# lgen-sudo/EgoM2P

Measured on AMD Instinct MI355X. Metric: multimodal tokens/sec (ego-b 400M, 10300-tok clips), training fwd+bwd+allreduce+AdamW, higher is better.
Workload: dtype bf16; 1 GPU; egom2p_base_12e_12d_swiglu_nobias mod4, synthetic 10300-position clips (1009+1009 rgb, 1009+1009 depth, 15+15 cam, 15+15 gaze kept -> N=M=2048), bf16 MFMA GEMM/attention, fp32 residual/LN/CE/AdamW; micro_batch=64, global_batch=256, parallelism=dp1

## Files before the change

egom2p_amd/csrc/gemm.hip:

```cpp
#include "common.h"
#include "egom2p_hip.h"

namespace {

constexpr int BM = 128, BN = 128, BK = 64;
constexpr int TILE_BYTES = BM * BK * 2;
constexpr int STAGE_BYTES = 2 * TILE_BYTES;
constexpr int GEMM_LDS = 2 * STAGE_BYTES;
constexpr int EPI_BYTES = 16 * 1024;
constexpr int NT_LDS = GEMM_LDS + EPI_BYTES;

struct NTArgs {
    const bf16_t* A; long lda;
    const bf16_t* B; long ldb;
    void* C; long ldc;
    const float* R; long ldr;
    const float* bias;
    const int* m_range;
    int M, N, K, epi;
    const bf16_t* X; long ldx;
    bf16_t* H; long ldh;
    const float* sa; const float* sb;
    int dephase;
};
// ... 124 lines not shown
                    for (int i = 0; i < 4; ++i) {
                        const int ml = i * 16 + (lane & 15);
#pragma unroll
                        for (int j = 0; j < 4; ++j) {
                            const int c = wn * 16 + j * 4 + (lane >> 4);
                            *(f32x4*)(ebuf + ml * 512 + ((c ^ (ml & 15)) << 4)) = acc[i][j];
                        }
                    }
                }
                lds_barrier();
#pragma unroll
                for (int ps = 0; ps < 8; ++ps) {
                    const int r = ps * 8 + (tid >> 5), c = tid & 31;
                    f32x4 v = *(const f32x4*)(ebuf + r * 512 + ((c ^ (r & 15)) << 4));
                    const int gm = row0 + half * 64 + r, gn = col0 + c * 4;
                    if (gm < M && gn < p.N) {
                        const long mrow = moff + gm;
                        if (p.epi == EGO_EPI_RESID) {
                            const f32x4 rr = *(const f32x4*)(p.R + mrow * p.ldr + gn);
                            v = f32x4{rr[0] + round_bf16(v[0]), rr[1] + round_bf16(v[1]), rr[2] + round_bf16(v[2]), rr[3] + round_bf16(v[3])};
                        } else if (p.epi == EGO_EPI_BIAS_RESID) {
                            const f32x4 rr = *(const f32x4*)(p.R + mrow * p.ldr + gn);
                            const f32x4 b = *(const f32x4*)(p.bias + gn);
                            v = f32x4{rr[0] + round_bf16(v[0] + round_bf16(b[0])), rr[1] + round_bf16(v[1] + round_bf16(b[1])),
                                      rr[2] + round_bf16(v[2] + round_bf16(b[2])), rr[3] + round_bf16(v[3] + round_bf16(b[3]))};
                        }
                        *(f32x4*)((float*)p.C + mrow * p.ldc + gn) = v;
                    }
                }
                lds_barrier();
            }
        }
        if (!more) break;
        tile = next_tile;
    }
}

template <int TM, int TN, int NS>
struct NTL {
    static constexpr int PA = TM / 32, PB = TN / 32;
    static constexpr int TA = TM * 128, TB = TN * 128;
    static constexpr int STAGE = TA + TB;
    static constexpr int LDS = NS * STAGE;
    static constexpr int PER = PA + PB;
};
constexpr int NT64_LDS = NTL<64, 64, 4>::LDS;
constexpr int NTL128x64_LDS = NTL<128, 64, 3>::LDS;
constexpr int NTL128x128_LDS = NTL<128, 128, 3>::LDS;

template <int N>
__device__ __forceinline__ void vm_wait() { asm volatile("s_waitcnt vmcnt(%0)" ::"n"(N) : "memory"); }

template <int TM, int TN, int NS>
__global__ __launch_bounds__(256, (NTL<TM, TN, NS>::LDS <= 80 * 1024 ? 2 : 1)) void gemm_ntl_kernel(NTArgs p) {
    using T = NTL<TM, TN, NS>;
    constexpr int MI = TM / 32, NI = TN / 32;
    extern __shared__ __attribute__((aligned(16))) char smem[];
    const int tid = threadIdx.x, lane = tid & 63;
    const int wave = __builtin_amdgcn_readfirstlane(tid >> 6);
    const int wm = wave >> 1, wn = wave & 1;
    int M = p.M;
    long moff = 0;
    if (p.m_range) { moff = p.m_range[0]; M = min(M, p.m_range[1]); }
    const int tiles_n = (p.N + TN - 1) / TN;
    const int tile = xcd_remap(blockIdx.x, gridDim.x);
    const int row0 = (tile / tiles_n) * TM, col0 = (tile % tiles_n) * TN;
    if (row0 >= M) return;
    const int nt = p.K / BK;

    const bf16_t* ga[T::PA];
    const bf16_t* gb[T::PB];
#pragma unroll
    for (int j = 0; j < T::PA; ++j) {
        const int r = 8 * (T::PA * wave + j) + (lane >> 3);
        ga[j] = p.A + (moff + min(row0 + r, M - 1)) * p.lda + ((lane & 7) ^ (r & 7)) * 8;
    }
#pragma unroll
    for (int j = 0; j < T::PB; ++j) {
        const int r = 8 * (T::PB * wave + j) + (lane >> 3);
        gb[j] = p.B + (long)min(col0 + r, p.N - 1) * p.ldb + ((lane & 7) ^ (r & 7)) * 8;
    }
    auto stage = [&](int s, int k0) {
        char* sa = smem + s * T::STAGE + wave * T::PA * 1024;
        char* sb = smem + s * T::STAGE + T::TA + wave * T::PB * 1024;
#pragma unroll
        for (int j = 0; j < T::PA; ++j) glds16(ga[j] + k0, sa + j * 1024);
#pragma unroll
        for (int j = 0; j < T::PB; ++j) glds16(gb[j] + k0, sb + j * 1024);
    };
#pragma unroll
    for (int s = 0; s < NS - 1; ++s)
        if (s < nt) stage(s, s * BK);

    f32x4 acc[MI][NI];
#pragma unroll
    for (int i = 0; i < MI; ++i)
#pragma unroll
        for (int j = 0; j < NI; ++j) acc[i][j] = f32x4{0.f, 0.f, 0.f, 0.f};
    int cur = 0;
    for (int kt = 0; kt < nt; ++kt) {
        const int younger = min(nt - 1 - kt, NS - 2);
        if (NS >= 4 && younger >= 2) vm_wait<2 * T::PER>();
        else if (younger >= 1) vm_wait<T::PER>();
        else vm_wait<0>();
        lds_barrier();
        if (kt + NS - 1 < nt) stage(cur == 0 ? NS - 1 : cur - 1, (kt + NS - 1) * BK);
        const char* sa = smem + cur * T::STAGE;
        const char* sb = sa + T::TA;
#pragma unroll
        for (int ks = 0; ks < 2; ++ks) {
            bf16x8 af[MI], bfr[NI];
            const int c = ks * 4 + (lane >> 4);
#pragma unroll
            for (int i = 0; i < MI; ++i) {
                const int ar = wm * (TM / 2) + i * 16 + (lane & 15);
                af[i] = *(const bf16x8*)(sa + ar * 128 + ((c ^ (ar & 7)) << 4));
            }
#pragma unroll
            for (int j = 0; j < NI; ++j) {
                const int br = wn * (TN / 2) + j * 16 + (lane & 15);
                bfr[j] = *(const bf16x8*)(sb + br * 128 + ((c ^ (br & 7)) << 4));
            }
#pragma unroll
            for (int i = 0; i < MI; ++i)
#pragma unroll
                for (int j = 0; j < NI; ++j)
                    acc[i][j] = __builtin_amdgcn_mfma_f32_16x16x32_bf16(bfr[j], af[i], acc[i][j], 0, 0, 0);
        }
        cur = (cur + 1 == NS) ? 0 : cur + 1;
    }

#pragma unroll
    for (int i = 0; i < MI; ++i) {
        const int gm = row0 + wm * (TM / 2) + i * 16 + (lane & 15);
#pragma unroll
        for (int j = 0; j < NI; ++j) {
            const int gn = col0 + wn * (TN / 2) + j * 16 + 4 * (lane >> 4);
            if (gm >= M || gn >= p.N) continue;
            const long mrow = moff + gm;
            f32x4 v = acc[i][j];
            if (p.epi == EGO_EPI_BF16) {
                *(u32x2*)((bf16_t*)p.C + mrow * p.ldc + gn) = u32x2{pack_bf16x2(v[0], v[1]), pack_bf16x2(v[2], v[3])};
                continue;
            }
            if (p.epi == EGO_EPI_RESID) {
                const f32x4 rr = *(const f32x4*)(p.R + mrow * p.ldr + gn);
                v = f32x4{rr[0] + round_bf16(v[0]), rr[1] + round_bf16(v[1]), rr[2] + round_bf16(v[2]), rr[3] + round_bf16(v[3])};
            } else if (p.epi == EGO_EPI_BIAS_RESID) {
                const f32x4 rr = *(const f32x4*)(p.R + mrow * p.ldr + gn);
                const f32x4 b = *(const f32x4*)(p.bias + gn);
                v = f32x4{rr[0] + round_bf16(v[0] + round_bf16(b[0])), rr[1] + round_bf16(v[1] + round_bf16(b[1])),
                          rr[2] + round_bf16(v[2] + round_bf16(b[2])), rr[3] + round_bf16(v[3] + round_bf16(b[3]))};
            }
            *(f32x4*)((float*)p.C + mrow * p.ldc + gn) = v;
        }
    }
}
#define gemm_nt64_kernel (gemm_ntl_kernel<64, 64, 4>)

constexpr int T2_BYTES = 256 * 128;
constexpr int S2_BYTES = 2 * T2_BYTES;
constexpr int NT2_LDS = 2 * S2_BYTES;

__device__ __forceinline__ void bar_pinned() {
    __builtin_amdgcn_sched_barrier(0);
    __builtin_amdgcn_s_barrier();
    __builtin_amdgcn_sched_barrier(0);
}

#ifndef NT256_STRIPS
#define NT256_STRIPS 1
#endif
#ifndef NT256_A_AUX
#define NT256_A_AUX 0
#endif
#ifndef NT256_B_AUX
#define NT256_B_AUX 0
#endif
constexpr int RA_BYTES = 256 * 128;
constexpr int NT3_LDS = 5 * RA_BYTES;

typedef int i32x8 __attribute__((ext_vector_type(8)));
__device__ __forceinline__ i32x8 cat_frag(bf16x8 lo, bf16x8 hi) {
    typedef int i32x4 __attribute__((ext_vector_type(4)));
    const i32x4 a = __builtin_bit_cast(i32x4, lo), b = __builtin_bit_cast(i32x4, hi);
    return __builtin_shufflevector(a, b, 0, 1, 2, 3, 4, 5, 6, 7);
}

template <int EK, bool FP8 = false, bool STRIPS = false>
__global__ __launch_bounds__(512, 2) void gemm_nt256_kernel(NTArgs p) {
    constexpr int ESZ = FP8 ? 1 : 2;
    extern __shared__ __attribute__((aligned(16))) char smem[];
    const int tid = threadIdx.x, lane = tid & 63;
    const int wave = __builtin_amdgcn_readfirstlane(tid >> 6);
    const int grp = wave >> 2, wc = wave & 3;

    int M = p.M;
    long moff = 0;
    if (p.m_range) { moff = p.m_range[0]; M = min(M, p.m_range[1]); }
    if (M <= 0) return;
    const int tiles_n = EK == 3 ? p.N / 128 : (p.N + 255) / 256;
    const int tile_w = EK == 3 ? 128 : 256;
    const int ntiles = ((M + 255) / 256) * tiles_n;
    if ((int)blockIdx.x >= ntiles) return;
    const int nt = p.K * ESZ / 128;
    const int G = gridDim.x;
    if (p.dephase > 0 && ((blockIdx.x >> 3) & 1))
        for (int i = 0; i < p.dephase; ++i) __builtin_amdgcn_s_sleep(16);

    auto a_rsrc = [&](int row0) {
        return __builtin_amdgcn_make_buffer_rsrc((void*)((const char*)p.A + (moff + row0) * p.lda * ESZ), 0,
                                                 (int)(unsigned)((long)(min(256, M - row0) - 1) * p.lda * ESZ + (long)p.K * ESZ), 0x00020000);
    };
    const __amdgpu_buffer_rsrc_t brs = __builtin_amdgcn_make_buffer_rsrc(
        (void*)p.B, 0, (int)(unsigned)((long)((EK == 3 ? 2 * p.N : p.N) - 1) * p.ldb * ESZ + (long)p.K * ESZ), 0x00020000);
    unsigned a_off0, b_off0;
    {
        const int r = 8 * (wave * 4) + (lane >> 3), c = ((lane & 7) ^ (r & 7)) * 16;
        a_off0 = (unsigned)(r * (int)p.lda * ESZ + c);
        b_off0 = (unsigned)((EK == 3 && r >= 128 ? p.N - 128 + r : r) * (int)p.ldb * ESZ + c);
    }
    const unsigned a_step = (unsigned)(8 * (int)p.lda * ESZ), b_step = (unsigned)(8 * (int)p.ldb * ESZ);
    const int rows_t = (M + 255) / 256;
    const int nstrips = STRIPS ? (tiles_n + 7) / 8 : 1;
    const int w0 = tiles_n / nstrips, wide = tiles_n % nstrips;
    const int big = wide * (w0 + 1) * rows_t;
    auto tile_origin = [&](int id, int& row0, int& col0) {
        const int t = xcd_remap(id, ntiles);
        int tr, tc;
        if constexpr (STRIPS) {
            int rem, w, c0;
            if (t < big) { const int per = (w0 + 1) * rows_t, sidx = t / per; rem = t - sidx * per; w = w0 + 1; c0 = sidx * (w0 + 1); }
            else { const int per = w0 * rows_t, u = t - big, sidx = u / per; rem = u - sidx * per; w = w0; c0 = wide * (w0 + 1) + sidx * w0; }
            tr = rem / w; tc = c0 + rem % w;
        } else {
            tr = t / tiles_n; tc = t % tiles_n;
        }
        row0 = tr * 256; col0 = tc * tile_w;
    };
    int idA = blockIdx.x, ktA = 0, rA, cA_unused, slotA = 0; bool moreA = true;
    int idB = blockIdx.x, ktB = 0, rB_unused, cB, slotB = 0; bool moreB = true;
    tile_origin(idA, rA, cA_unused);
    tile_origin(idB, rB_unused, cB);
    unsigned a_so = 0, b_so = 0;
    __amdgpu_buffer_rsrc_t ars = a_rsrc(rA);
    auto cursorA = [&]() { a_so = (unsigned)(ktA * BK * 2); };
    auto advanceA = [&]() {
        slotA = slotA == 2 ? 0 : slotA + 1;
        if (++ktA == nt) {
            ktA = 0; idA += G;
            if (idA < ntiles) { tile_origin(idA, rA, cA_unused); ars = a_rsrc(rA); } else moreA = false;
        }
    };
    auto cursorB = [&]() { b_so = (unsigned)cB * (unsigned)(p.ldb * ESZ) + (unsigned)(ktB * BK * 2); };
    auto advanceB = [&]() {
        slotB ^= 1;
        if (++ktB == nt) { ktB = 0; idB += G; if (idB < ntiles) tile_origin(idB, rB_unused, cB); else moreB = false; }
    };
    auto dmaA = [&](int slot, int j) {
        __builtin_amdgcn_raw_ptr_buffer_load_lds(ars, (__attribute__((address_space(3))) void*)(smem + slot * RA_BYTES + (wave * 4 + j) * 1024),
                                                 16, a_off0, (int)(a_so + j * a_step), 0, NT256_A_AUX);
    };
    auto dmaB = [&](int slot, int j) {
        __builtin_amdgcn_raw_ptr_buffer_load_lds(brs, (__attribute__((address_space(3))) void*)(smem + (3 + slot) * RA_BYTES + (wave * 4 + j) * 1024),
                                                 16, b_off0, (int)(b_so + j * b_step), 0, NT256_B_AUX);
    };
#ifndef FP8_FRAG_OLD
#define FP8_FRAG_OLD 0
#endif
    int foff[2];
#pragma unroll
    for (int ks = 0; ks < 2; ++ks)
        foff[ks] = (lane & 15) * 128 + ((((FP8 && FP8_FRAG_OLD) ? 2 * (lane >> 4) + ks : ks * 4 + (lane >> 4)) ^ (lane & 7)) << 4);
    const int a_base = grp * 128 * 128, b_base = wc * 64 * 128;

    int id = blockIdx.x, row0, col0;
    tile_origin(id, row0, col0);
    cursorA();
#pragma unroll
    for (int j = 0; j < 4; ++j) dmaA(slotA, j);
    advanceA();
    cursorB();
#pragma unroll
    for (int j = 0; j < 4; ++j) dmaB(slotB, j);
    advanceB();
    if (moreA) {
        cursorA();
#pragma unroll
        for (int j = 0; j < 4; ++j) dmaA(slotA, j);
        advanceA();
        asm volatile("s_waitcnt vmcnt(4)" ::: "memory");
    } else {
        asm volatile("s_waitcnt vmcnt(0)" ::: "memory");
    }
    bar_pinned();
    int curA = 0, curB = 0;

#define LOAD_A(QM)                                                                                         \
    _Pragma("unroll") for (int mi = 0; mi < 4; ++mi) _Pragma("unroll") for (int ks = 0; ks < 2; ++ks)      \
        af[mi][ks] = *(const bf16x8*)(sa + a_base + ((QM) * 4 + mi) * 2048 + foff[ks]);
#define LOAD_B(QN)                                                                                         \
    _Pragma("unroll") for (int ni = 0; ni < 2; ++ni) _Pragma("unroll") for (int ks = 0; ks < 2; ++ks)      \
        bq[ni][ks] = *(const bf16x8*)(sb + b_base + ((QN) * 2 + ni) * 2048 + foff[ks]);
#define COMPUTE(QM, QN)                                                                                    \
    __builtin_amdgcn_s_setprio(1);                                                                         \
    if constexpr (FP8) {                                                                                   \
        _Pragma("unroll") for (int mi = 0; mi < 4; ++mi) _Pragma("unroll") for (int ni = 0; ni < 2; ++ni)  \
            acc[(QM) * 4 + mi][(QN) * 2 + ni] = __builtin_amdgcn_mfma_scale_f32_16x16x128_f8f6f4(          \
                cat_frag(bq[ni][0], bq[ni][1]), cat_frag(af[mi][0], af[mi][1]),                            \
                acc[(QM) * 4 + mi][(QN) * 2 + ni], 0, 0, 0, 127, 0, 127);                                  \
    } else {                                                                                               \
        _Pragma("unroll") for (int ks = 0; ks < 2; ++ks) _Pragma("unroll") for (int mi = 0; mi < 4; ++mi)  \
            _Pragma("unroll") for (int ni = 0; ni < 2; ++ni)                                               \
                acc[(QM) * 4 + mi][(QN) * 2 + ni] = __builtin_amdgcn_mfma_f32_16x16x32_bf16(               \
                    bq[ni][ks], af[mi][ks], acc[(QM) * 4 + mi][(QN) * 2 + ni], 0, 0, 0);                   \
    }                                                                                                      \
    __builtin_amdgcn_s_setprio(0);

    while (true) {
        f32x4 acc[8][4];
#pragma unroll
        for (int i = 0; i < 8; ++i)
#pragma unroll
            for (int j = 0; j < 4; ++j) acc[i][j] = f32x4{0.f, 0.f, 0.f, 0.f};
        bf16x8 af[4][2], bq[2][2];

        if (grp == 1) bar_pinned();
        for (int kt = 0; kt < nt; ++kt) {
            const char* sa = smem + curA * RA_BYTES;
            const char* sb = smem + (3 + curB) * RA_BYTES;
            const bool fa = moreA, fb = moreB;
            const int sA = slotA, sB = slotB;
            if (fa) cursorA();
            if (fb) cursorB();
            LOAD_A(0) LOAD_B(0)
            if (grp == 1) { if (fb) { dmaB(sB, 0); dmaB(sB, 1); } } else if (fa) { dmaA(sA, 0); dmaA(sA, 1); }
            bar_pinned();
            COMPUTE(0, 0)
            bar_pinned();
            LOAD_B(1)
            if (fb) { if (grp == 1) { dmaB(sB, 2); dmaB(sB, 3); } else { dmaB(sB, 0); dmaB(sB, 1); } }
            bar_pinned();
            COMPUTE(0, 1)
            bar_pinned();
            LOAD_A(1)
            if (grp == 1) { if (fa) { dmaA(sA, 0); dmaA(sA, 1); } } else if (fb) { dmaB(sB, 2); dmaB(sB, 3); }
            bar_pinned();
            COMPUTE(1, 1)
            bar_pinned();
            LOAD_B(0)
            if (fa) { dmaA(sA, 2); dmaA(sA, 3); }
            if (grp == 1) { if (fa) asm volatile("s_waitcnt vmcnt(4)" ::: "memory"); else asm volatile("s_waitcnt vmcnt(0)" ::: "memory"); }
            bar_pinned();
            COMPUTE(1, 0)
            if (grp == 0) { if (fa) asm volatile("s_waitcnt vmcnt(2)" ::: "memory"); else asm volatile("s_waitcnt vmcnt(0)" ::: "memory"); }
            bar_pinned();
            if (fa) advanceA();
            if (fb) advanceB();
            curA = curA == 2 ? 0 : curA + 1;
            curB ^= 1;
        }
        if (grp == 0) bar_pinned();
        asm volatile("s_waitcnt lgkmcnt(0)" ::: "memory");

        char* ea = smem + (curA == 0 ? 2 : curA - 1) * RA_BYTES;
        char* ebb = smem + (3 + (curB ^ 1)) * RA_BYTES;
        if constexpr (FP8) {
            float ra[8];
            f32x4 cb[4];
#pragma unroll
            for (int i = 0; i < 8; ++i) ra[i] = p.sa[moff + min(row0 + grp * 128 + i * 16 + (lane & 15), M - 1)];
#pragma unroll
            for (int j = 0; j < 4; ++j) {
                const int tc = wc * 64 + j * 16 + (lane >> 4) * 4;
                const int bn = EK == 3 ? (tc < 128 ? col0 + tc : p.N + col0 + tc - 128) : min(col0 + tc, p.N - 4);
                cb[j] = *(const f32x4*)(p.sb + bn);
            }
#pragma unroll
            for (int j = 0; j < 4; ++j)
#pragma unroll
                for (int i = 0; i < 8; ++i) acc[i][j] = acc[i][j] * (cb[j] * ra[i]);
        }
        if constexpr (EK == 0) {
#pragma unroll
            for (int half = 0; half < 2; ++half) {
                if (grp == half) {
    #pragma unroll
                    for (int i = 0; i < 8; ++i) {
                        const int ml = i * 16 + (lane & 15);
                        char* eb = (i < 4 ? ea : ebb) + (ml & 63) * 512;
    #pragma unroll
                        for (int j = 0; j < 4; ++j) {
                            const int slot = wc * 16 + j * 4 + (lane >> 4);
                            const f32x4 v = acc[i][j];
                            u32x2 o = {pack_bf16x2(v[0], v[1]), pack_bf16x2(v[2], v[3])};
                            *(u32x2*)(eb + (((slot >> 1) ^ (ml & 15)) << 4) + (slot & 1) * 8) = o;
                        }
                    }
                }
                lds_barrier();
    #pragma unroll
                for (int ps = 0; ps < 8; ++ps) {
                    const int r = ps * 16 + (tid >> 5), c = tid & 31;
                    const u32x4 v = *(const u32x4*)((ps < 4 ? ea : ebb) + (r & 63) * 512 + ((c ^ (r & 15)) << 4));
                    const int gm = row0 + half * 128 + r, gn = col0 + c * 8;
                    if (gm < M && gn < p.N) __builtin_nontemporal_store(v, (u32x4*)((bf16_t*)p.C + (moff + gm) * p.ldc + gn));
                }
                lds_barrier();
            }
        } else if constexpr (EK == 3) {
            bf16_t* Cb = (bf16_t*)p.C + moff * p.ldc;
            bf16_t* Hb = p.H + moff * p.ldh;
#pragma unroll
            for (int half = 0; half < 2; ++half) {
                if (grp == half) {
#pragma unroll
                    for (int i = 0; i < 8; ++i) {
                        const int ml = i * 16 + (lane & 15);
                        char* eb = (i < 4 ? ea : ebb) + (ml & 63) * 512;
#pragma unroll
                        for (int j = 0; j < 4; ++j) {
                            const int slot = wc * 16 + j * 4 + (lane >> 4);
                            const f32x4 v = acc[i][j];
                            u32x2 o = {pack_bf16x2(v[0], v[1]), pack_bf16x2(v[2], v[3])};
                            *(u32x2*)(eb + (((slot >> 1) ^ (ml & 15)) << 4) + (slot & 1) * 8) = o;
                        }
                    }
                }
                lds_barrier();
#pragma unroll
                for (int ps = 0; ps < 4; ++ps) {
                    const int r = ps * 32 + (tid >> 4), c = tid & 15;
                    const char* rowp = (ps < 2 ? ea : ebb) + (r & 63) * 512;
                    const u32x4 av = *(const u32x4*)(rowp + ((c ^ (r & 15)) << 4));
                    const u32x4 bv = *(const u32x4*)(rowp + (((c + 16) ^ (r & 15)) << 4));
                    u32x4 hv;
#pragma unroll
                    for (int e = 0; e < 4; ++e) {
                        const float a0 = bf16_to_f32(av[e] & 0xffff), a1 = bf16_to_f32(av[e] >> 16);
                        const float b0 = bf16_to_f32(bv[e] & 0xffff), b1 = bf16_to_f32(bv[e] >> 16);
                        hv[e] = pack_bf16x2(round_bf16(a0 * sigmoidf_(a0)) * b0, round_bf16(a1 * sigmoidf_(a1)) * b1);
                    }
                    const int gm = row0 + half * 128 + r, gn = col0 + c * 8;
                    if (gm < M) {
                        __builtin_nontemporal_store(av, (u32x4*)(Cb + (long)gm * p.ldc + gn));
                        __builtin_nontemporal_store(bv, (u32x4*)(Cb + (long)gm * p.ldc + p.N + gn));
                        __builtin_nontemporal_store(hv, (u32x4*)(Hb + (long)gm * p.ldh + gn));
                    }
                }
                lds_barrier();
            }
        } else if constexpr (EK == 2) {
            const bf16_t* Xb = p.X + moff * p.ldx;
            bf16_t* Yb = (bf16_t*)p.C + moff * p.ldc;
            auto load_ab = [&](int g, u32x4 (&av)[2], u32x4 (&bv)[2]) {
#pragma unroll
                for (int k = 0; k < 2; ++k) {
                    const int gm = row0 + (g >> 2) * 128 + ((g & 3) * 2 + k) * 16 + (tid >> 5), gn = col0 + (tid & 31) * 8;
                    const u32x4 z = {0u, 0u, 0u, 0u};
                    const bool ok = g < 8 && gm < M;
                    av[k] = ok ? __builtin_nontemporal_load((const u32x4*)(Xb + (long)gm * p.ldx + gn)) : z;
                    bv[k] = ok ? __builtin_nontemporal_load((const u32x4*)(Xb + (long)gm * p.ldx + p.N + gn)) : z;
                }
            };
            auto process = [&](int g, const u32x4 (&av)[2], const u32x4 (&bv)[2]) {
#pragma unroll
                for (int k = 0; k < 2; ++k) {
                    const int ps = (g & 3) * 2 + k;
                    const int r = ps * 16 + (tid >> 5), c = tid & 31;
                    const u32x4 gq = *(const u32x4*)((ps < 4 ? ea : ebb) + (r & 63) * 512 + ((c ^ (r & 15)) << 4));
                    const int gm = row0 + (g >> 2) * 128 + r, gn = col0 + c * 8;
                    u32x4 oa, ob;
#pragma unroll
                    for (int e = 0; e < 4; ++e) {
                        const float a2[2] = {bf16_to_f32(av[k][e] & 0xffff), bf16_to_f32(av[k][e] >> 16)};
                        const float b2[2] = {bf16_to_f32(bv[k][e] & 0xffff), bf16_to_f32(bv[k][e] >> 16)};
                        const float g2[2] = {bf16_to_f32(gq[e] & 0xffff), bf16_to_f32(gq[e] >> 16)};
                        float da[2], db[2];
#pragma unroll
                        for (int t = 0; t < 2; ++t) {
                            const float sg = sigmoidf_(a2[t]);
                            da[t] = g2[t] * b2[t] * sg * (1.f + a2[t] * (1.f - sg));
                            db[t] = g2[t] * a2[t] * sg;
                        }
                        oa[e] = pack_bf16x2(da[0], da[1]);
                        ob[e] = pack_bf16x2(db[0], db[1]);
                    }
                    if (gm < M) {
                        __builtin_nontemporal_store(oa, (u32x4*)(Yb + (long)gm * p.ldc + gn));
                        __builtin_nontemporal_store(ob, (u32x4*)(Yb + (long)gm * p.ldc + p.N + gn));
                    }
                }
            };
            u32x2 pk[8][4];
#pragma unroll
            for (int i = 0; i < 8; ++i)
#pragma unroll
                for (int j = 0; j < 4; ++j) {
                    const f32x4 v = acc[i][j];
                    pk[i][j] = u32x2{pack_bf16x2(v[0], v[1]), pack_bf16x2(v[2], v[3])};
                }
            u32x4 av[4][2], bv[4][2];
#pragma unroll
            for (int g = 0; g < 4; ++g) load_ab(g, av[g], bv[g]);
#pragma unroll
            for (int half = 0; half < 2; ++half) {
                if (grp == half) {
#pragma unroll
                    for (int i = 0; i < 8; ++i) {
                        const int ml = i * 16 + (lane & 15);
                        char* eb = (i < 4 ? ea : ebb) + (ml & 63) * 512;
#pragma unroll
                        for (int j = 0; j < 4; ++j) {
                            const int slot = wc * 16 + j * 4 + (lane >> 4);
                            *(u32x2*)(eb + (((slot >> 1) ^ (ml & 15)) << 4) + (slot & 1) * 8) = pk[i][j];
                        }
                    }
                }
                lds_barrier();
#pragma unroll
                for (int gg = 0; gg < 4; ++gg) {
                    const int g = half * 4 + gg;
                    process(g, av[gg], bv[gg]);
                    if (half == 0) load_ab(g + 4, av[gg], bv[gg]);
                }
                lds_barrier();
            }
        } else {
            const bool has_r = (p.epi == EGO_EPI_RESID || p.epi == EGO_EPI_BIAS_RESID);
            f32x4 bb = {0.f, 0.f, 0.f, 0.f};
            if (p.epi == EGO_EPI_BIAS_RESID) {
                const int gn = col0 + (tid & 63) * 4;
                if (gn < p.N) { const f32x4 b = *(const f32x4*)(p.bias + gn); bb = f32x4{round_bf16(b[0]), round_bf16(b[1]), round_bf16(b[2]), round_bf16(b[3])}; }
            }
            auto load_r = [&](int q, int hb, f32x4 (&rr)[4]) {
#pragma unroll
                for (int k = 0; k < 4; ++k) {
                    const int gm = row0 + q * 64 + (hb * 4 + k) * 8 + (tid >> 6), gn = col0 + (tid & 63) * 4;
                    rr[k] = (has_r && q < 4 && gm < M && gn < p.N) ? __builtin_nontemporal_load((const f32x4*)(p.R + (moff + gm) * p.ldr + gn))
                                                                    : f32x4{0.f, 0.f, 0.f, 0.f};
                }
            };
            f32x4 rlo[4], rhi[4];
            load_r(0, 0, rlo);
            load_r(0, 1, rhi);
#pragma unroll
            for (int q = 0; q < 4; ++q) {
                if (grp == (q >> 1)) {
#pragma unroll
                    for (int ii = 0; ii < 4; ++ii) {
                        const int i = (q & 1) * 4 + ii;
                        const int ml = ii * 16 + (lane & 15);
                        char* eb = (ii < 2 ? ea : ebb) + (ml & 31) * 1024;
#pragma unroll
                        for (int j = 0; j < 4; ++j) {
                            const int c = wc * 16 + j * 4 + (lane >> 4);
                            *(f32x4*)(eb + ((c ^ (ml & 15)) << 4)) = acc[i][j];
                        }
                    }
                }
                lds_barrier();
#pragma unroll
                for (int hb = 0; hb < 2; ++hb) {
                    f32x4 (&rr)[4] = hb == 0 ? rlo : rhi;
#pragma unroll
                    for (int k = 0; k < 4; ++k) {
                        const int r = (hb * 4 + k) * 8 + (tid >> 6), c = tid & 63;
                        f32x4 v = *(const f32x4*)((hb == 0 ? ea : ebb) + (r & 31) * 1024 + ((c ^ (r & 15)) << 4));
                        const int gm = row0 + q * 64 + r, gn = col0 + c * 4;
                        if (gm < M && gn < p.N) {
                            if (has_r) {
                                const f32x4 x = rr[k];
                                v = f32x4{x[0] + round_bf16(v[0] + bb[0]), x[1] + round_bf16(v[1] + bb[1]),
                                          x[2] + round_bf16(v[2] + bb[2]), x[3] + round_bf16(v[3] + bb[3])};
                            }
                            *(f32x4*)((float*)p.C + (moff + gm) * p.ldc + gn) = v;
                        }
                    }
                    if (q < 3) load_r(q + 1, hb, rr);
                }
                lds_barrier();
            }
        }
        id += G;
        if (id >= ntiles) break;
        tile_origin(id, row0, col0);
    }
#undef LOAD_A
#undef LOAD_B
#undef COMPUTE
}

struct TNArgs {
    const bf16_t* P; long ldp;
    const bf16_t* Q; long ldq;
    float* C0; float* C1; long ldc;
    float* slab;
    const int* m_range;
    int split_row, rows0, rows1;
    int Ni, Nj, M, splits;
};

__device__ __forceinline__ int tn_f(int r) { return (r & 3) | (((r >> 3) & 1) << 2); }


template <int S>
__device__ __forceinline__ void tn_compute(const unsigned (&pb)[4], const unsigned (&qb)[4], f32x4 (&acc)[4][4]) {
    constexpr int O = S * STAGE_BYTES;
    s16x4 p0[4][2], q0[4][2], p1[4][2], q1[4][2];
#pragma unroll
    for (int i = 0; i < 4; ++i) {
        p0[i][0] = tr_read<O>(pb[i]);              p0[i][1] = tr_read<O + 1024>(pb[i]);
        q0[i][0] = tr_read<O + TILE_BYTES>(qb[i]); q0[i][1] = tr_read<O + TILE_BYTES + 1024>(qb[i]);
    }
    asm volatile("s_waitcnt lgkmcnt(0)" ::: "memory");
    __builtin_amdgcn_sched_barrier(0);
#pragma unroll
    for (int i = 0; i < 4; ++i) {
        p1[i][0] = tr_read<O + 8192>(pb[i]);              p1[i][1] = tr_read<O + 8192 + 1024>(pb[i]);
        q1[i][0] = tr_read<O + TILE_BYTES + 8192>(qb[i]); q1[i][1] = tr_read<O + TILE_BYTES + 8192 + 1024>(qb[i]);
    }
    __builtin_amdgcn_sched_barrier(0);
#pragma unroll
    for (int i = 0; i < 4; ++i)
#pragma unroll
        for (int j = 0; j < 4; ++j)
            acc[i][j] = __builtin_amdgcn_mfma_f32_16x16x32_bf16(join8(q0[j][0], q0[j][1]), join8(p0[i][0], p0[i][1]), acc[i][j], 0, 0, 0);
    __builtin_amdgcn_sched_barrier(0);
    asm volatile("s_waitcnt lgkmcnt(0)" ::: "memory");
    __builtin_amdgcn_sched_barrier(0);
#pragma unroll
    for (int i = 0; i < 4; ++i)
#pragma unroll
        for (int j = 0; j < 4; ++j)
            acc[i][j] = __builtin_amdgcn_mfma_f32_16x16x32_bf16(join8(q1[j][0], q1[j][1]), join8(p1[i][0], p1[i][1]), acc[i][j], 0, 0, 0);
}

__global__ __launch_bounds__(256, 2) void gemm_tn_kernel(TNArgs p) {
    extern __shared__ __attribute__((aligned(16))) char smem[];
    const int tid = threadIdx.x, lane = tid & 63;
    const int wave = __builtin_amdgcn_readfirstlane(tid >> 6);
    const int wi = wave >> 1, wj = wave & 1;

    int M = p.M;
    long moff = 0;
    if (p.m_range) { moff = p.m_range[0]; M = min(M, p.m_range[1]); }
    const int tiles_j = p.Nj / BN, tiles_i = p.Ni / BM;
    const int ntile = tiles_i * tiles_j;
    const int bid = blockIdx.x;
    const int split = bid / ntile;
    const int t = xcd_remap(bid % ntile, ntile);
    const int i0 = (t / tiles_j) * BM, j0 = (t % tiles_j) * BN;

    const int nsteps = (M + BK - 1) / BK;
    const int per = (nsteps + p.splits - 1) / p.splits;
    const int st0 = split * per, st1 = min(nsteps, st0 + per);

    const bf16_t* P = p.P + moff * p.ldp + i0;
    const bf16_t* Q = p.Q + moff * p.ldq + j0;

    long p_off[4], q_off[4];
#pragma unroll
    for (int j = 0; j < 4; ++j) {
        const int r = 4 * (wave * 4 + j) + (lane >> 4), s16 = lane & 15;
        const int c = (((s16 >> 1) ^ tn_f(r)) << 1) | (s16 & 1);
// ... 488 lines not shown
```

Measured before the change: 1.964 million clip-positions/s.

## Interleave LDS reads and DMA issues between individual MFMAs in bf16 GEMM mainloop

For the bf16 path, the GEMM mainloop is rewritten as a hand-scheduled sequence. Each MFMA is followed by one LDS fragment read or global-to-LDS DMA issue, with sched_barrier pins between them. The next tile's first fragments are prefetched during the last quarter, and there are fewer workgroup barriers per k-step. The aim is to hide LDS latency and barrier stalls behind matrix math. This risks correctness hazards from the changed wait counts and barrier placement, plus extra register pressure. The FP8 path keeps the old loop.

```diff
diff --git a/egom2p_amd/csrc/gemm.hip b/egom2p_amd/csrc/gemm.hip
--- a/egom2p_amd/csrc/gemm.hip
+++ b/egom2p_amd/csrc/gemm.hip
@@ -450,20 +450,23 @@
 #define LOAD_B(QN)                                                                                         \
     _Pragma("unroll") for (int ni = 0; ni < 2; ++ni) _Pragma("unroll") for (int ks = 0; ks < 2; ++ks)      \
         bq[ni][ks] = *(const bf16x8*)(sb + b_base + ((QN) * 2 + ni) * 2048 + foff[ks]);
-#define COMPUTE(QM, QN)                                                                                    \
+#define COMPUTE(QM, QN)                          \
     __builtin_amdgcn_s_setprio(1);                                                                         \
-    if constexpr (FP8) {                                                                                   \
-        _Pragma("unroll") for (int mi = 0; mi < 4; ++mi) _Pragma("unroll") for (int ni = 0; ni < 2; ++ni)  \
-            acc[(QM) * 4 + mi][(QN) * 2 + ni] = __builtin_amdgcn_mfma_scale_f32_16x16x128_f8f6f4(          \
-                cat_frag(bq[ni][0], bq[ni][1]), cat_frag(af[mi][0], af[mi][1]),                            \
-                acc[(QM) * 4 + mi][(QN) * 2 + ni], 0, 0, 0, 127, 0, 127);                                  \
-    } else {                                                                                               \
-        _Pragma("unroll") for (int ks = 0; ks < 2; ++ks) _Pragma("unroll") for (int mi = 0; mi < 4; ++mi)  \
-            _Pragma("unroll") for (int ni = 0; ni < 2; ++ni)                                               \
-                acc[(QM) * 4 + mi][(QN) * 2 + ni] = __builtin_amdgcn_mfma_f32_16x16x32_bf16(               \
-                    bq[ni][ks], af[mi][ks], acc[(QM) * 4 + mi][(QN) * 2 + ni], 0, 0, 0);                   \
-    }                                                                                                      \
+    _Pragma("unroll") for (int mi = 0; mi < 4; ++mi) _Pragma("unroll") for (int ni = 0; ni < 2; ++ni)      \
+        acc[(QM) * 4 + mi][(QN) * 2 + ni] = __builtin_amdgcn_mfma_scale_f32_16x16x128_f8f6f4(              \
+            cat_frag(bq[ni][0], bq[ni][1]), cat_frag(af[mi][0], af[mi][1]),                                \
+            acc[(QM) * 4 + mi][(QN) * 2 + ni], 0, 0, 0, 127, 0, 127);                                      \
     __builtin_amdgcn_s_setprio(0);
+
+#define MF(QM, QN, KS, MI, NI)                                                                             \
+    acc[(QM) * 4 + (MI)][(QN) * 2 + (NI)] = __builtin_amdgcn_mfma_f32_16x16x32_bf16(                       \
+        bq[NI][KS], af[MI][KS], acc[(QM) * 4 + (MI)][(QN) * 2 + (NI)], 0, 0, 0);
+#define RD_A(S, QM, MI, KS) af[MI][KS] = *(const bf16x8*)((S) + a_base + ((QM) * 4 + (MI)) * 2048 + foff[KS]);
+#define RD_B(S, QN, NI, KS) bq[NI][KS] = *(const bf16x8*)((S) + b_base + ((QN) * 2 + (NI)) * 2048 + foff[KS]);
+#define PIN __builtin_amdgcn_sched_barrier(0);
+#define HALF(QM, QN, KS, U0, U1, U2, U3, U4, U5, U6, U7)                                                   \
+    MF(QM, QN, KS, 0, 0) U0 PIN MF(QM, QN, KS, 0, 1) U1 PIN MF(QM, QN, KS, 1, 0) U2 PIN MF(QM, QN, KS, 1, 1) U3 PIN \
+    MF(QM, QN, KS, 2, 0) U4 PIN MF(QM, QN, KS, 2, 1) U5 PIN MF(QM, QN, KS, 3, 0) U6 PIN MF(QM, QN, KS, 3, 1) U7 PIN
 
     while (true) {
         f32x4 acc[8][4];
@@ -473,42 +476,85 @@
             for (int j = 0; j < 4; ++j) acc[i][j] = f32x4{0.f, 0.f, 0.f, 0.f};
         bf16x8 af[4][2], bq[2][2];
 
-        if (grp == 1) bar_pinned();
-        for (int kt = 0; kt < nt; ++kt) {
-            const char* sa = smem + curA * RA_BYTES;
-            const char* sb = smem + (3 + curB) * RA_BYTES;
-            const bool fa = moreA, fb = moreB;
-            const int sA = slotA, sB = slotB;
-            if (fa) cursorA();
-            if (fb) cursorB();
-            LOAD_A(0) LOAD_B(0)
-            if (grp == 1) { if (fb) { dmaB(sB, 0); dmaB(sB, 1); } } else if (fa) { dmaA(sA, 0); dmaA(sA, 1); }
-            bar_pinned();
-            COMPUTE(0, 0)
-            bar_pinned();
-            LOAD_B(1)
-            if (fb) { if (grp == 1) { dmaB(sB, 2); dmaB(sB, 3); } else { dmaB(sB, 0); dmaB(sB, 1); } }
-            bar_pinned();
-            COMPUTE(0, 1)
-            bar_pinned();
-            LOAD_A(1)
-            if (grp == 1) { if (fa) { dmaA(sA, 0); dmaA(sA, 1); } } else if (fb) { dmaB(sB, 2); dmaB(sB, 3); }
-            bar_pinned();
-            COMPUTE(1, 1)
-            bar_pinned();
-            LOAD_B(0)
-            if (fa) { dmaA(sA, 2); dmaA(sA, 3); }
-            if (grp == 1) { if (fa) asm volatile("s_waitcnt vmcnt(4)" ::: "memory"); else asm volatile("s_waitcnt vmcnt(0)" ::: "memory"); }
-            bar_pinned();
-            COMPUTE(1, 0)
-            if (grp == 0) { if (fa) asm volatile("s_waitcnt vmcnt(2)" ::: "memory"); else asm volatile("s_waitcnt vmcnt(0)" ::: "memory"); }
-            bar_pinned();
-            if (fa) advanceA();
-            if (fb) advanceB();
-            curA = curA == 2 ? 0 : curA + 1;
-            curB ^= 1;
-        }
-        if (grp == 0) bar_pinned();
+        if constexpr (FP8) {
+            if (grp == 1) bar_pinned();
+            for (int kt = 0; kt < nt; ++kt) {
+                const char* sa = smem + curA * RA_BYTES;
+                const char* sb = smem + (3 + curB) * RA_BYTES;
+                const bool fa = moreA, fb = moreB;
+                const int sA = slotA, sB = slotB;
+                if (fa) cursorA();
+                if (fb) cursorB();
+                LOAD_A(0) LOAD_B(0)
+                if (grp == 1) { if (fb) { dmaB(sB, 0); dmaB(sB, 1); } } else if (fa) { dmaA(sA, 0); dmaA(sA, 1); }
+                bar_pinned();
+                COMPUTE(0, 0)
+                bar_pinned();
+                LOAD_B(1)
+                if (fb) { if (grp == 1) { dmaB(sB, 2); dmaB(sB, 3); } else { dmaB(sB, 0); dmaB(sB, 1); } }
+                bar_pinned();
+                COMPUTE(0, 1)
+                bar_pinned();
+                LOAD_A(1)
+                if (grp == 1) { if (fa) { dmaA(sA, 0); dmaA(sA, 1); } } else if (fb) { dmaB(sB, 2); dmaB(sB, 3); }
+                bar_pinned();
+                COMPUTE(1, 1)
+                bar_pinned();
+                LOAD_B(0)
+                if (fa) { dmaA(sA, 2); dmaA(sA, 3); }
+                if (grp == 1) { if (fa) asm volatile("s_waitcnt vmcnt(4)" ::: "memory"); else asm volatile("s_waitcnt vmcnt(0)" ::: "memory"); }
+                bar_pinned();
+                COMPUTE(1, 0)
+                if (grp == 0) { if (fa) asm volatile("s_waitcnt vmcnt(2)" ::: "memory"); else asm volatile("s_waitcnt vmcnt(0)" ::: "memory"); }
+                bar_pinned();
+                if (fa) advanceA();
+                if (fb) advanceB();
+                curA = curA == 2 ? 0 : curA + 1;
+                curB ^= 1;
+            }
+            if (grp == 0) bar_pinned();
+        } else {
+            {
+                const char* sa = smem + curA * RA_BYTES;
+                const char* sb = smem + (3 + curB) * RA_BYTES;
+                RD_A(sa, 0, 0, 0) RD_B(sb, 0, 0, 0) RD_B(sb, 0, 1, 0) RD_A(sa, 0, 1, 0) RD_A(sa, 0, 2, 0) RD_A(sa, 0, 3, 0)
+            }
+            for (int kt = 0; kt < nt; ++kt) {
+                const int nxtA = curA == 2 ? 0 : curA + 1;
+                const char* sa = smem + curA * RA_BYTES;
+                const char* sb = smem + (3 + curB) * RA_BYTES;
+                const char* sa_n = smem + nxtA * RA_BYTES;
+                const char* sb_n = smem + (3 + (curB ^ 1)) * RA_BYTES;
+                const bool fa = moreA, fb = moreB;
+                const int sA = slotA, sB = slotB;
+                if (fa) cursorA();
+                if (fb) cursorB();
+                PIN
+                HALF(0, 0, 0, RD_A(sa, 0, 0, 1), RD_B(sb, 0, 0, 1), RD_B(sb, 0, 1, 1), RD_A(sa, 0, 1, 1), RD_A(sa, 0, 2, 1), RD_A(sa, 0, 3, 1),
+                     if (fb) dmaB(sB, 0);, )
+                HALF(0, 0, 1, RD_B(sb, 1, 0, 0), RD_B(sb, 1, 1, 0), , if (fb) dmaB(sB, 1);, , if (fb) dmaB(sB, 2);, , )
+                bar_pinned();
+                HALF(0, 1, 0, RD_B(sb, 1, 0, 1), RD_B(sb, 1, 1, 1), , if (fb) dmaB(sB, 3);, , , if (fa) dmaA(sA, 0);, )
+                HALF(0, 1, 1, RD_A(sa, 1, 0, 0), RD_A(sa, 1, 1, 0), RD_A(sa, 1, 2, 0), RD_A(sa, 1, 3, 0), , , , )
+                bar_pinned();
+                HALF(1, 1, 0, RD_A(sa, 1, 0, 1), RD_A(sa, 1, 1, 1), RD_A(sa, 1, 2, 1), RD_A(sa, 1, 3, 1), , if (fa) dmaA(sA, 1);, , )
+                HALF(1, 1, 1, RD_B(sb, 0, 0, 0), RD_B(sb, 0, 1, 0), , if (fa) dmaA(sA, 2);, , , , )
+                if (fa) asm volatile("s_waitcnt vmcnt(3)" ::: "memory"); else asm volatile("s_waitcnt vmcnt(0)" ::: "memory");
+                bar_pinned();
+                HALF(1, 0, 0, RD_B(sb, 0, 0, 1), RD_B(sb, 0, 1, 1), , if (fa) dmaA(sA, 3);, , , , )
+                if (kt + 1 < nt) {
+                    HALF(1, 0, 1, RD_A(sa_n, 0, 0, 0), RD_B(sb_n, 0, 0, 0), RD_B(sb_n, 0, 1, 0), RD_A(sa_n, 0, 1, 0), RD_A(sa_n, 0, 2, 0),
+                         RD_A(sa_n, 0, 3, 0), , )
+                } else {
+                    HALF(1, 0, 1, , , , , , , , )
+                }
+                bar_pinned();
+                if (fa) advanceA();
+                if (fb) advanceB();
+                curA = nxtA;
+                curB ^= 1;
+            }
+        }
         asm volatile("s_waitcnt lgkmcnt(0)" ::: "memory");
 
         char* ea = smem + (curA == 0 ? 2 : curA - 1) * RA_BYTES;
```

Measured after the change: 1.966 million clip-positions/s (median of 2 runs). About the same (+0.1%).
